# naver-ai/egtr

Measured on AMD Instinct MI355X. Metric: images/sec end-to-end SGG, 600x1000 input, N=200 queries, higher is better.
Workload: dtype f32; 1 GPU; VG inference: ResNet-50, N=200, 6 enc/6 dec, 150 classes, 50 predicates, 600x1000, bs=1/GPU fp32 (BASELINE configs[1]); hip_graph=True, gemm_tuning=True, miopen_find=True, parallelism=replicas x1 (independent images, no collective)

## Files before the change

### egtr_amd/csrc/conv3x3_x6.hip

```cpp
#include <hip/hip_runtime.h>
#include <stdint.h>

#include "common.h"
#include "x6_common.h"
#include "xs_format.h"

namespace {
using namespace x6;
typedef float f32x4v __attribute__((ext_vector_type(4)));

__device__ __forceinline__ f32x4v shift_relu(f32x4v v, f32x4v sh) {
  return f32x4v{egtr_relu(v.x + sh.x), egtr_relu(v.y + sh.y), egtr_relu(v.z + sh.z), egtr_relu(v.w + sh.w)};
}

struct ConvArgs {
  const float* x;
  const char* w;
  float* y;
  int B, H, W, N;
  int tiles_x, tiles_y;
  const float* in_shift;
};

#ifdef EGTR_CONV_TIMING
constexpr int kRecWg = 4096;
__device__ unsigned long long g_conv_rec[kRecWg][8];
#define CONV_T(v) const unsigned long long v = __builtin_amdgcn_s_memtime()
#else
#define CONV_T(v) do { } while (0)
#endif

template <int C, int TH, int WM, int NTW, int NWV = 4, bool SHIFT = false>
__global__ __launch_bounds__(64 * NWV) void conv3x3_x6_kernel(ConvArgs A) {
  constexpr int TW = 8;
  constexpr int HW_ = TW + 2, HH = TH + 2, HP = HH * HW_;
  constexpr int KC = C / 16;
  constexpr int KS = 9 * KC;
  constexpr int kPitch = C + 8;
  constexpr int MTW = (TH / 4) / WM;
  constexpr int WN = NWV / WM;
  constexpr int NT = 64 * NWV;
  constexpr int BN = 32 * NTW * WN;
#ifndef EGTR_CONV_PF
#define EGTR_CONV_PF 3
#endif
  constexpr int PF = EGTR_CONV_PF;
  constexpr int C4 = C / 4;
  static_assert(TH % (4 * WM) == 0 && NWV % WM == 0, "tile shape");
  extern __shared__ __attribute__((aligned(16))) char s_raw[];
  __bf16* const sA = reinterpret_cast<__bf16*>(s_raw);

  const int tid = threadIdx.x, lane = tid & 63, li = lane & 31, hf = lane >> 5;
  const int wave = __builtin_amdgcn_readfirstlane(tid >> 6);
  const int wm = wave / WN, wn = wave % WN;
#ifdef EGTR_CONV_TIMING
  const unsigned long long rt0 = __builtin_amdgcn_s_memrealtime();
#endif
  CONV_T(t0);
  const int nblocks = A.N / BN;
  int t = blockIdx.x;
  const int nb = t % nblocks;
  t /= nblocks;
  const int tx = t % A.tiles_x;
  t /= A.tiles_x;
  const int ty = t % A.tiles_y, b = t / A.tiles_y;
  const int y0 = ty * TH, x0 = tx * TW;
  const int nt0 = nb * (BN / 32) + wn * NTW;

  const char* const wlane = A.w + (size_t)nt0 * KS * (3 * xs::kFragBytes) + lane * 16;
  bf16x8 w[PF + 1][NTW][3];
  auto load_w = [&](int ks, bf16x8 (&dst)[NTW][3]) {
#pragma unroll
    for (int tt = 0; tt < NTW; ++tt)
#pragma unroll
      for (int p = 0; p < 3; ++p)
        dst[tt][p] = *reinterpret_cast<const bf16x8*>(wlane + ((size_t)(tt * KS + ks) * 3 + p) * xs::kFragBytes);
  };

  {
    constexpr float kPad = SHIFT ? -__builtin_inff() : 0.f;
    static_assert(!SHIFT || NT % C4 == 0, "one channel quad per thread");
    f32x4v sh = f32x4v{0.f, 0.f, 0.f, 0.f};
    if constexpr (SHIFT) sh = *reinterpret_cast<const f32x4v*>(A.in_shift + 4 * (tid % C4));
    constexpr int CHUNKS = HP * C4;
    constexpr int NQ = (CHUNKS + NT - 1) / NT;
    constexpr int CH = 6;
    const float* const xb = A.x + (size_t)b * A.H * A.W * C;
#pragma unroll
    for (int q0 = 0; q0 < NQ; q0 += CH) {
      f32x4v v[CH];
#pragma unroll
      for (int q = 0; q < CH; ++q) {
        const int idx = tid + NT * (q0 + q);
        const int hp = idx / C4, c4 = idx % C4;
        const int gy = y0 - 1 + hp / HW_, gx = x0 - 1 + hp % HW_;
        const bool in = (q0 + q < NQ) && idx < CHUNKS && gy >= 0 && gy < A.H && gx >= 0 && gx < A.W;
        v[q] = f32x4v{kPad, kPad, kPad, kPad};
        if (in) v[q] = *reinterpret_cast<const f32x4v*>(xb + ((size_t)gy * A.W + gx) * C + 4 * c4);
      }
      if (q0 == 0) {
        static_for<PF>([&](auto i_) {
          constexpr int i = decltype(i_)::value;
          load_w(i, w[i]);
        });
        __builtin_amdgcn_sched_barrier(0);
      }
#pragma unroll
      for (int q = 0; q < CH; ++q) {
        const int idx = tid + NT * (q0 + q);
        if (q0 + q < NQ && idx < CHUNKS) {
          const int hp = idx / C4, c4 = idx % C4;
          f32x4v u = v[q];
          if constexpr (SHIFT) u = shift_relu(u, sh);
          const xs::Split3 s0 = xs::split3_fast(u.x), s1 = xs::split3_fast(u.y), s2 = xs::split3_fast(u.z),
                           s3 = xs::split3_fast(u.w);
          __bf16* p = sA + hp * kPitch + 4 * c4;
          *reinterpret_cast<uint2*>(p) = make_uint2(xs::pack_hi16(s0.hi, s1.hi), xs::pack_hi16(s2.hi, s3.hi));
          *reinterpret_cast<uint2*>(p + HP * kPitch) = make_uint2(xs::pack_hi16(s0.mid, s1.mid), xs::pack_hi16(s2.mid, s3.mid));
          *reinterpret_cast<uint2*>(p + 2 * HP * kPitch) = make_uint2(xs::pack_hi16(s0.lo, s1.lo), xs::pack_hi16(s2.lo, s3.lo));
        }
      }
    }
  }
  CONV_T(t1);
  __syncthreads();
  CONV_T(t2);

  f32x16 acc[MTW][NTW];
#pragma unroll
  for (int m = 0; m < MTW; ++m)
#pragma unroll
    for (int tt = 0; tt < NTW; ++tt)
#pragma unroll
      for (int r = 0; r < 16; ++r) acc[m][tt][r] = 0.f;

  const __bf16* pa[MTW];
#pragma unroll
  for (int m = 0; m < MTW; ++m)
    pa[m] = sA + ((4 * (wm * MTW + m) + (li >> 3)) * HW_ + (li & 7)) * kPitch + 8 * hf;
  bf16x8 a[2][MTW][3];
  auto read_a = [&](auto ks_, bf16x8 (&dst)[MTW][3]) {
    constexpr int ks = decltype(ks_)::value;
    constexpr int tap = ks / KC, kc = ks % KC;
    constexpr int off = ((tap / 3) * HW_ + (tap % 3)) * kPitch + 16 * kc;
#pragma unroll
    for (int m = 0; m < MTW; ++m)
#pragma unroll
      for (int p = 0; p < 3; ++p) dst[m][p] = *reinterpret_cast<const bf16x8*>(pa[m] + p * HP * kPitch + off);
  };
  read_a(std::integral_constant<int, 0>{}, a[0]);
  static_for<KS>([&](auto ks_) {
    constexpr int ks = decltype(ks_)::value;
    if constexpr (ks + PF < KS) load_w(ks + PF, w[(ks + PF) % (PF + 1)]);
    if constexpr (ks + 1 < KS) read_a(std::integral_constant<int, ks + 1>{}, a[(ks + 1) & 1]);
    __builtin_amdgcn_sched_barrier(0);
#pragma unroll
    for (int m = 0; m < MTW; ++m)
#pragma unroll
      for (int tt = 0; tt < NTW; ++tt) acc[m][tt] = mfma6(a[ks & 1][m], w[ks % (PF + 1)][tt], acc[m][tt]);
    __builtin_amdgcn_sched_barrier(0);
  });

  CONV_T(t3);
  float* const yb = A.y + (size_t)b * A.H * A.W * A.N;
#pragma unroll
  for (int m = 0; m < MTW; ++m)
#pragma unroll
    for (int tt = 0; tt < NTW; ++tt) {
      const int col = (nt0 + tt) * 32 + li;
#pragma unroll
      for (int r = 0; r < 16; ++r) {
        const int p = (r & 3) + 8 * (r >> 2) + 4 * hf;
        const int gy = y0 + 4 * (wm * MTW + m) + (p >> 3), gx = x0 + (p & 7);
        if (gy < A.H && gx < A.W) yb[((size_t)gy * A.W + gx) * A.N + col] = acc[m][tt][r];
      }
    }
#ifdef EGTR_CONV_TIMING
  CONV_T(t4);
  asm volatile("s_waitcnt vmcnt(0)" ::: "memory");
  CONV_T(t5);
  if (tid == 0 && blockIdx.x < kRecWg) {
    unsigned long long* r = g_conv_rec[blockIdx.x];
    r[0] = rt0;
    r[1] = __builtin_amdgcn_s_memrealtime();
    r[2] = t1 - t0;
    r[3] = t2 - t1;
    r[4] = t3 - t2;
    r[5] = t4 - t3;
    r[6] = t5 - t4;
    r[7] = 1;
  }
#endif
}

template <int C, int CP, int STRIDE, int TAPS = 9, bool SHIFT = false>
__global__ __launch_bounds__(256) void conv3x3_x6_phased_kernel(ConvArgs A) {
  constexpr int TH = 4, TW = 8;
  static_assert(TAPS == 9 || TAPS == 1, "3x3 or 1x1");
  constexpr int HH = TAPS == 9 ? STRIDE * (TH - 1) + 3 : TH, HW_ = TAPS == 9 ? STRIDE * (TW - 1) + 3 : TW, HP = HH * HW_;
  constexpr int PH = C / CP;
  constexpr int KCP = CP / 16;
  constexpr int KSP = TAPS * KCP;
  constexpr int KS = PH * KSP;
  constexpr int kPitch = CP + 8;
  constexpr int PF = EGTR_CONV_PF;
  constexpr int C4 = CP / 4;
  static_assert(KSP % (PF + 1) == 0, "the fragment ring must line up at the phase boundary");
  static_assert(!SHIFT || (TAPS == 9 && 256 % C4 == 0), "one channel quad per thread");
  extern __shared__ __attribute__((aligned(16))) char s_raw[];
  __bf16* const sA = reinterpret_cast<__bf16*>(s_raw);

  const int tid = threadIdx.x, lane = tid & 63, li = lane & 31, hf = lane >> 5;
  const int wave = __builtin_amdgcn_readfirstlane(tid >> 6);
  const int nblocks = A.N / 128;
  int t = blockIdx.x;
  const int nb = t % nblocks;
  t /= nblocks;
  const int tx = t % A.tiles_x;
  t /= A.tiles_x;
  const int ty = t % A.tiles_y, b = t / A.tiles_y;
  const int y0 = ty * TH, x0 = tx * TW;
  const int iy0 = STRIDE * y0 - 1, ix0 = STRIDE * x0 - 1;
  const int nt = nb * 4 + wave;

  const char* const wlane = A.w + (size_t)nt * KS * (3 * xs::kFragBytes) + lane * 16;
  bf16x8 w[PF + 1][3];
  auto load_w = [&](int ks, bf16x8 (&dst)[3]) {
#pragma unroll
    for (int p = 0; p < 3; ++p) dst[p] = *reinterpret_cast<const bf16x8*>(wlane + ((size_t)ks * 3 + p) * xs::kFragBytes);
  };
  static_for<PF>([&](auto i_) {
    constexpr int i = decltype(i_)::value;
    load_w(i, w[i]);
  });
  __builtin_amdgcn_sched_barrier(0);

  f32x16 acc;
#pragma unroll
  for (int r = 0; r < 16; ++r) acc[r] = 0.f;
  const float* const xb = A.x + (size_t)b * A.H * A.W * C;
  constexpr int PS = TAPS == 9 ? STRIDE : 1;
  const __bf16* const pa = sA + (PS * (li >> 3) * HW_ + PS * (li & 7)) * kPitch + 8 * hf;

#pragma unroll 1
  for (int ph = 0; ph < PH; ++ph) {
    if (ph > 0) __syncthreads();
    {
      constexpr int CHUNKS = HP * C4;
      constexpr int NQ = (CHUNKS + 255) / 256;
      constexpr int CH = NQ < 8 ? NQ : 8;
      constexpr float kPad = SHIFT ? -__builtin_inff() : 0.f;
      f32x4v sh = f32x4v{0.f, 0.f, 0.f, 0.f};
      if constexpr (SHIFT) sh = *reinterpret_cast<const f32x4v*>(A.in_shift + ph * CP + 4 * (tid % C4));
#pragma unroll
      for (int q0 = 0; q0 < NQ; q0 += CH) {
        f32x4v v[CH];
#pragma unroll
        for (int q = 0; q < CH; ++q) {
          const int idx = tid + 256 * (q0 + q);
          const int hp = idx / C4, c4 = idx % C4;
          const int gy = TAPS == 9 ? iy0 + hp / HW_ : STRIDE * (y0 + hp / HW_), gx = TAPS == 9 ? ix0 + hp % HW_ : STRIDE * (x0 + hp % HW_);
          const bool in = (q0 + q < NQ) && idx < CHUNKS && gy >= 0 && gy < A.H && gx >= 0 && gx < A.W;
          v[q] = f32x4v{kPad, kPad, kPad, kPad};
          if (in) v[q] = *reinterpret_cast<const f32x4v*>(xb + ((size_t)gy * A.W + gx) * C + ph * CP + 4 * c4);
        }
#pragma unroll
        for (int q = 0; q < CH; ++q) {
          const int idx = tid + 256 * (q0 + q);
          if (q0 + q < NQ && idx < CHUNKS) {
            const int hp = idx / C4, c4 = idx % C4;
            f32x4v u = v[q];
            if constexpr (SHIFT) u = shift_relu(u, sh);
            const xs::Split3 s0 = xs::split3_fast(u.x), s1 = xs::split3_fast(u.y), s2 = xs::split3_fast(u.z),
                             s3 = xs::split3_fast(u.w);
            __bf16* p = sA + hp * kPitch + 4 * c4;
            *reinterpret_cast<uint2*>(p) = make_uint2(xs::pack_hi16(s0.hi, s1.hi), xs::pack_hi16(s2.hi, s3.hi));
            *reinterpret_cast<uint2*>(p + HP * kPitch) = make_uint2(xs::pack_hi16(s0.mid, s1.mid), xs::pack_hi16(s2.mid, s3.mid));
            *reinterpret_cast<uint2*>(p + 2 * HP * kPitch) = make_uint2(xs::pack_hi16(s0.lo, s1.lo), xs::pack_hi16(s2.lo, s3.lo));
          }
        }
      }
    }
    __syncthreads();

    const int ks0 = ph * KSP;
    bf16x8 a[2][3];
    auto read_a = [&](auto j_, bf16x8 (&dst)[3]) {
      constexpr int j = decltype(j_)::value;
      constexpr int tap = j / KCP, kc = j % KCP;
      constexpr int off = ((tap / 3) * HW_ + (tap % 3)) * kPitch + 16 * kc;
#pragma unroll
      for (int p = 0; p < 3; ++p) dst[p] = *reinterpret_cast<const bf16x8*>(pa + p * HP * kPitch + off);
    };
    read_a(std::integral_constant<int, 0>{}, a[0]);
    static_for<KSP>([&](auto j_) {
      constexpr int j = decltype(j_)::value;
      if (ks0 + j + PF < KS) load_w(ks0 + j + PF, w[(j + PF) % (PF + 1)]);
      if constexpr (j + 1 < KSP) read_a(std::integral_constant<int, j + 1>{}, a[(j + 1) & 1]);
      __builtin_amdgcn_sched_barrier(0);
      acc = mfma6(a[j & 1], w[j % (PF + 1)], acc);
      __builtin_amdgcn_sched_barrier(0);
    });
  }

  const int Ho = (A.H - 1) / STRIDE + 1, Wo = (A.W - 1) / STRIDE + 1;
  float* const yb = A.y + (size_t)b * Ho * Wo * A.N;
  const int col = nt * 32 + li;
#pragma unroll
  for (int r = 0; r < 16; ++r) {
    const int p = (r & 3) + 8 * (r >> 2) + 4 * hf;
    const int gy = y0 + (p >> 3), gx = x0 + (p & 7);
    if (gy < Ho && gx < Wo) yb[((size_t)gy * Wo + gx) * A.N + col] = acc[r];
  }
}

template <int C, int CP, int STRIDE, bool SHIFT = false>
__global__ __launch_bounds__(256) void conv3x3_x6_ksplit_kernel(ConvArgs A) {
  constexpr int TH = 4, TW = 8;
  constexpr int HH = STRIDE * (TH - 1) + 3, HW_ = STRIDE * (TW - 1) + 3, HP = HH * HW_;
  constexpr int PH = C / CP;
  constexpr int KCP = CP / 16;
  constexpr int KSP = 9 * KCP;
  constexpr int KCW = KCP / 4;
  constexpr int JS = 9 * KCW;
  constexpr int kPitch = CP + 8;
  constexpr int PF = (JS % 6 == 0) ? 5 : 2;
  constexpr int C4 = CP / 4;
  static_assert(KCP % 4 == 0 && JS % (PF + 1) == 0, "phase shape");
  static_assert(!SHIFT || 256 % C4 == 0, "one channel quad per thread");
  extern __shared__ __attribute__((aligned(16))) char s_raw[];
  __bf16* const sA = reinterpret_cast<__bf16*>(s_raw);

  const int tid = threadIdx.x, lane = tid & 63, li = lane & 31, hf = lane >> 5;
  const int wave = __builtin_amdgcn_readfirstlane(tid >> 6);
  const int ntiles = A.N / 32;
  int t = blockIdx.x;
  const int nt = t % ntiles;
  t /= ntiles;
  const int tx = t % A.tiles_x;
  t /= A.tiles_x;
  const int ty = t % A.tiles_y, b = t / A.tiles_y;
  const int y0 = ty * TH, x0 = tx * TW;
  const int iy0 = STRIDE * y0 - 1, ix0 = STRIDE * x0 - 1;

  const char* const wlane = A.w + (size_t)nt * (PH * KSP) * (3 * xs::kFragBytes) + lane * 16;
  auto wptr = [&](int ph, int j) {
    const int ks = ph * KSP + (j / KCW) * KCP + wave * KCW + (j % KCW);
    return wlane + (size_t)ks * 3 * xs::kFragBytes;
  };
  bf16x8 w[PF + 1][3];
  auto load_w = [&](int ph, int j, bf16x8 (&dst)[3]) {
    const char* p0 = wptr(ph, j);
#pragma unroll
    for (int p = 0; p < 3; ++p) dst[p] = *reinterpret_cast<const bf16x8*>(p0 + p * xs::kFragBytes);
  };
  static_for<PF>([&](auto i_) {
    constexpr int i = decltype(i_)::value;
    load_w(0, i, w[i]);
  });
  __builtin_amdgcn_sched_barrier(0);

  f32x16 acc;
#pragma unroll
  for (int r = 0; r < 16; ++r) acc[r] = 0.f;
  const float* const xb = A.x + (size_t)b * A.H * A.W * C;
  const __bf16* const pa = sA + (STRIDE * (li >> 3) * HW_ + STRIDE * (li & 7)) * kPitch + 8 * hf + 16 * KCW * wave;

#pragma unroll 1
  for (int ph = 0; ph < PH; ++ph) {
    if (ph > 0) __syncthreads();
    {
      constexpr int CHUNKS = HP * C4;
      constexpr int NQ = (CHUNKS + 255) / 256;
      constexpr int CH = NQ < 8 ? NQ : 8;
      constexpr float kPad = SHIFT ? -__builtin_inff() : 0.f;
      f32x4v sh = f32x4v{0.f, 0.f, 0.f, 0.f};
      if constexpr (SHIFT) sh = *reinterpret_cast<const f32x4v*>(A.in_shift + ph * CP + 4 * (tid % C4));
#pragma unroll
      for (int q0 = 0; q0 < NQ; q0 += CH) {
        f32x4v v[CH];
#pragma unroll
        for (int q = 0; q < CH; ++q) {
          const int idx = tid + 256 * (q0 + q);
          const int hp = idx / C4, c4 = idx % C4;
          const int gy = iy0 + hp / HW_, gx = ix0 + hp % HW_;
          const bool in = (q0 + q < NQ) && idx < CHUNKS && gy >= 0 && gy < A.H && gx >= 0 && gx < A.W;
          v[q] = f32x4v{kPad, kPad, kPad, kPad};
          if (in) v[q] = *reinterpret_cast<const f32x4v*>(xb + ((size_t)gy * A.W + gx) * C + ph * CP + 4 * c4);
        }
#pragma unroll
        for (int q = 0; q < CH; ++q) {
          const int idx = tid + 256 * (q0 + q);
          if (q0 + q < NQ && idx < CHUNKS) {
            const int hp = idx / C4, c4 = idx % C4;
            f32x4v u = v[q];
            if constexpr (SHIFT) u = shift_relu(u, sh);
            const xs::Split3 s0 = xs::split3_fast(u.x), s1 = xs::split3_fast(u.y), s2 = xs::split3_fast(u.z),
                             s3 = xs::split3_fast(u.w);
            __bf16* p = sA + hp * kPitch + 4 * c4;
            *reinterpret_cast<uint2*>(p) = make_uint2(xs::pack_hi16(s0.hi, s1.hi), xs::pack_hi16(s2.hi, s3.hi));
            *reinterpret_cast<uint2*>(p + HP * kPitch) = make_uint2(xs::pack_hi16(s0.mid, s1.mid), xs::pack_hi16(s2.mid, s3.mid));
            *reinterpret_cast<uint2*>(p + 2 * HP * kPitch) = make_uint2(xs::pack_hi16(s0.lo, s1.lo), xs::pack_hi16(s2.lo, s3.lo));
          }
        }
      }
    }
    __syncthreads();

    bf16x8 a[2][3];
    auto read_a = [&](auto j_, bf16x8 (&dst)[3]) {
      constexpr int j = decltype(j_)::value;
      constexpr int tap = j / KCW, kcl = j % KCW;
      constexpr int off = ((tap / 3) * HW_ + (tap % 3)) * kPitch + 16 * kcl;
#pragma unroll
      for (int p = 0; p < 3; ++p) dst[p] = *reinterpret_cast<const bf16x8*>(pa + p * HP * kPitch + off);
    };
    read_a(std::integral_constant<int, 0>{}, a[0]);
    static_for<JS>([&](auto j_) {
      constexpr int j = decltype(j_)::value;
      if constexpr (j + PF < JS) {
        load_w(ph, j + PF, w[(j + PF) % (PF + 1)]);
      } else {
        if (ph + 1 < PH) load_w(ph + 1, j + PF - JS, w[(j + PF) % (PF + 1)]);
      }
      if constexpr (j + 1 < JS) read_a(std::integral_constant<int, j + 1>{}, a[(j + 1) & 1]);
      __builtin_amdgcn_sched_barrier(0);
      acc = mfma6(a[j & 1], w[j % (PF + 1)], acc);
      __builtin_amdgcn_sched_barrier(0);
    });
  }

  __syncthreads();
  float* const part = reinterpret_cast<float*>(s_raw);
#pragma unroll
  for (int r = 0; r < 16; ++r) part[(wave * 16 + r) * 64 + lane] = acc[r];
  __syncthreads();
  const int Ho = (A.H - 1) / STRIDE + 1, Wo = (A.W - 1) / STRIDE + 1;
  float* const yb = A.y + (size_t)b * Ho * Wo * A.N;
  const int col = nt * 32 + li;
#pragma unroll
  for (int rr = 0; rr < 4; ++rr) {
    const int r = 4 * wave + rr;
    const float v = ((part[(0 * 16 + r) * 64 + lane] + part[(1 * 16 + r) * 64 + lane]) + part[(2 * 16 + r) * 64 + lane]) +
                    part[(3 * 16 + r) * 64 + lane];
    const int p = (r & 3) + 8 * (r >> 2) + 4 * hf;
    const int gy = y0 + (p >> 3), gx = x0 + (p & 7);
    if (gy < Ho && gx < Wo) yb[((size_t)gy * Wo + gx) * A.N + col] = v;
  }
}

template <int C, int CP, int STRIDE, bool SHIFT = false>
int launch_ksplit(hipStream_t st, ConvArgs A) {
  static unsigned long long raised = 0;
  constexpr int HP = (STRIDE * 3 + 3) * (STRIDE * 7 + 3);
  constexpr int lds = 3 * HP * (CP + 8) * 2;
  static_assert(lds >= 4 * 16 * 64 * 4, "the partial tiles reuse the halo tile's LDS");
  auto kern = conv3x3_x6_ksplit_kernel<C, CP, STRIDE, SHIFT>;
  if (lds > 64 * 1024) {
    const int rc = egtr_raise_dynamic_lds(reinterpret_cast<const void*>(kern), lds, &raised);
    if (rc != EGTR_OK) return rc;
  }
  const int Ho = (A.H - 1) / STRIDE + 1, Wo = (A.W - 1) / STRIDE + 1;
  A.tiles_x = (Wo + 7) / 8;
  A.tiles_y = (Ho + 3) / 4;
  const long long wgs = (long long)A.B * A.tiles_x * A.tiles_y * (A.N / 32);
  if (wgs >= (1ll << 31)) return EGTR_E_UNSUPPORTED;
  hipLaunchKernelGGL(kern, dim3((unsigned)wgs), dim3(256), lds, st, A);
  return egtr_check_launch();
}

template <int C, int CP, int STRIDE, int TAPS = 9, bool SHIFT = false>
int launch_phased(hipStream_t st, ConvArgs A) {
  static unsigned long long raised = 0;
  constexpr int HP = TAPS == 9 ? (STRIDE * 3 + 3) * (STRIDE * 7 + 3) : 32;
  constexpr int lds = 3 * HP * (CP + 8) * 2;
  auto kern = conv3x3_x6_phased_kernel<C, CP, STRIDE, TAPS, SHIFT>;
  if (lds > 64 * 1024) {
    const int rc = egtr_raise_dynamic_lds(reinterpret_cast<const void*>(kern), lds, &raised);
    if (rc != EGTR_OK) return rc;
  }
  const int Ho = (A.H - 1) / STRIDE + 1, Wo = (A.W - 1) / STRIDE + 1;
  A.tiles_x = (Wo + 7) / 8;
  A.tiles_y = (Ho + 3) / 4;
  const long long wgs = (long long)A.B * A.tiles_x * A.tiles_y * (A.N / 128);
  if (wgs >= (1ll << 31)) return EGTR_E_UNSUPPORTED;
  hipLaunchKernelGGL(kern, dim3((unsigned)wgs), dim3(256), lds, st, A);
  return egtr_check_launch();
}

template <int C, int TH, int WM, int NTW, int NWV = 4, bool SHIFT = false>
int launch(hipStream_t st, ConvArgs A) {
  static unsigned long long raised = 0;
  constexpr int lds = 3 * (TH + 2) * 10 * (C + 8) * 2;
  constexpr int BN = 32 * NTW * (NWV / WM);
  auto kern = conv3x3_x6_kernel<C, TH, WM, NTW, NWV, SHIFT>;
  if (lds > 64 * 1024) {
    const int rc = egtr_raise_dynamic_lds(reinterpret_cast<const void*>(kern), lds, &raised);
    if (rc != EGTR_OK) return rc;
  }
  A.tiles_x = (A.W + 7) / 8;
  A.tiles_y = (A.H + TH - 1) / TH;
  const long long wgs = (long long)A.B * A.tiles_x * A.tiles_y * (A.N / BN);
  if (wgs >= (1ll << 31)) return EGTR_E_UNSUPPORTED;
  hipLaunchKernelGGL(kern, dim3((unsigned)wgs), dim3(64 * NWV), lds, st, A);
  return egtr_check_launch();
}

}

#ifdef EGTR_CONV_TIMING
extern "C" int egtr_conv3x3_stamps(unsigned long long* host_out, int reset) {
  if (hipMemcpyFromSymbol(host_out, HIP_SYMBOL(g_conv_rec), sizeof(unsigned long long) * kRecWg * 8) != hipSuccess)
    return EGTR_E_LAUNCH;
  if (reset) {
    void* p = nullptr;
    if (hipGetSymbolAddress(&p, HIP_SYMBOL(g_conv_rec)) != hipSuccess ||
        hipMemset(p, 0, sizeof(unsigned long long) * kRecWg * 8) != hipSuccess)
      return EGTR_E_LAUNCH;
  }
  return EGTR_OK;
}
#endif

extern "C" int egtr_conv3x3_phase_channels(int C, int N, int stride, int variant) {
  if (C != N) return 0;
  if (stride == 1) {
    if (C == 64 || C == 128) return C;
    if (C == 256) return variant == 3 ? 256 : 128;
    if (C == 512) return 128;
    return 0;
  }
  if (stride == 2) return (C == 128 || C == 256 || C == 512) ? 64 : 0;
  return 0;
}

namespace {
template <bool SHIFT>
int conv3x3_dispatch(hipStream_t st, ConvArgs A, int C, int stride, int variant) {
  if (stride == 2) {
    if (C == 128) return variant == 1 ? launch_ksplit<128, 64, 2, SHIFT>(st, A) : launch_phased<128, 64, 2, 9, SHIFT>(st, A);
    if (C == 256) return variant == 1 ? launch_ksplit<256, 64, 2, SHIFT>(st, A) : launch_phased<256, 64, 2, 9, SHIFT>(st, A);
    if (variant == 1) return launch_phased<512, 64, 2, 9, SHIFT>(st, A);
    return launch_ksplit<512, 64, 2, SHIFT>(st, A);
  }
  if (C == 64) {
    if (variant == 1) return launch<64, 8, 2, 1, 4, SHIFT>(st, A);
    if (variant == 2) return launch<64, 16, 2, 1, 4, SHIFT>(st, A);
    if (variant == 3) return launch<64, 16, 4, 1, 4, SHIFT>(st, A);
    if (variant == 4) return launch_ksplit<64, 64, 1, SHIFT>(st, A);
    return launch<64, 4, 1, 1, 2, SHIFT>(st, A);
  }
  if (C == 128) {
    if (variant == 1) return launch<128, 8, 2, 1, 4, SHIFT>(st, A);
    if (variant == 3) return launch<128, 16, 4, 1, 4, SHIFT>(st, A);
    if (variant == 4) return launch<128, 4, 1, 1, 2, SHIFT>(st, A);
    if (variant == 2) return launch<128, 4, 1, 1, 4, SHIFT>(st, A);
    return launch_ksplit<128, 128, 1, SHIFT>(st, A);
  }
  if (C == 256) {
    if (variant == 1) return launch_phased<256, 128, 1, 9, SHIFT>(st, A);
    if (variant == 3) return launch<256, 4, 1, 1, 4, SHIFT>(st, A);
    return launch_ksplit<256, 128, 1, SHIFT>(st, A);
  }
  if (variant == 1) return launch_phased<512, 128, 1, 9, SHIFT>(st, A);
  return launch_ksplit<512, 128, 1, SHIFT>(st, A);
}

int conv3x3_check(const float* x, const void* w_xs, const float* y, int B, int H, int W, int C, int N, int stride, int variant) {
  if (!x || !w_xs || !y || B <= 0 || H <= 0 || W <= 0 || C <= 0 || N <= 0) return EGTR_E_ARG;
  if ((reinterpret_cast<uintptr_t>(x) & 15) || (reinterpret_cast<uintptr_t>(y) & 15) || (reinterpret_cast<uintptr_t>(w_xs) & 15))
    return EGTR_E_UNSUPPORTED;
  if (egtr_conv3x3_phase_channels(C, N, stride, variant) == 0) return EGTR_E_UNSUPPORTED;
  return EGTR_OK;
}
}

extern "C" int egtr_conv3x3_x6_f32(egtr_stream_t stream, const float* x, const void* w_xs, float* y, int B, int H, int W, int C,
                                   int N, int stride, int variant) {
  const int rc = conv3x3_check(x, w_xs, y, B, H, W, C, N, stride, variant);
  if (rc != EGTR_OK) return rc;
  ConvArgs A{x, static_cast<const char*>(w_xs), y, B, H, W, N, 0, 0, nullptr};
  return conv3x3_dispatch<false>(static_cast<hipStream_t>(stream), A, C, stride, variant);
}

extern "C" int egtr_conv3x3_x6_shift_f32(egtr_stream_t stream, const float* x, const float* in_shift, const void* w_xs, float* y,
                                         int B, int H, int W, int C, int N, int stride, int variant) {
  if (!in_shift) return EGTR_E_ARG;
  const int rc = conv3x3_check(x, w_xs, y, B, H, W, C, N, stride, variant);
  if (rc != EGTR_OK) return rc;
  if (reinterpret_cast<uintptr_t>(in_shift) & 15) return EGTR_E_UNSUPPORTED;
  ConvArgs A{x, static_cast<const char*>(w_xs), y, B, H, W, N, 0, 0, in_shift};
  return conv3x3_dispatch<true>(static_cast<hipStream_t>(stream), A, C, stride, variant);
}

extern "C" int egtr_conv1x1_strided_x6_f32(egtr_stream_t stream, const float* x, const void* w_xs, float* y, int B, int H, int W,
                                           int C, int N, int stride) {
  if (!x || !w_xs || !y || B <= 0 || H <= 0 || W <= 0 || C <= 0 || N <= 0) return EGTR_E_ARG;
  if ((reinterpret_cast<uintptr_t>(x) & 15) || (reinterpret_cast<uintptr_t>(y) & 15) || (reinterpret_cast<uintptr_t>(w_xs) & 15) ||
      N % 128 || (stride != 1 && stride != 2))
    return EGTR_E_UNSUPPORTED;
  ConvArgs A{x, static_cast<const char*>(w_xs), y, B, H, W, N, 0, 0, nullptr};
  hipStream_t st = static_cast<hipStream_t>(stream);
  if (stride == 2) {
    if (C == 256) return launch_phased<256, 256, 2, 1>(st, A);
    if (C == 512) return launch_phased<512, 256, 2, 1>(st, A);
    if (C == 1024) return launch_phased<1024, 256, 2, 1>(st, A);
    return EGTR_E_UNSUPPORTED;
  }
  if (C == 256) return launch_phased<256, 256, 1, 1>(st, A);
  if (C == 512) return launch_phased<512, 256, 1, 1>(st, A);
  if (C == 1024) return launch_phased<1024, 256, 1, 1>(st, A);
  return EGTR_E_UNSUPPORTED;
}
```

Measured before the change: 409.0 images/sec.

## Prefetch next channel phase's halo tile into registers during MFMA products

In the phased and k-split 3x3 conv kernels, when there are several channel phases, the global loads for the next phase's input halo are now issued in registers, spread across the MFMA steps of the current phase. They are parked into LDS (split to bf16x3) only after the products finish, which hides global-load latency behind the compute. Out-of-bounds loads are made branch-free by reading from a device pad constant. Launch bounds now request several workgroups per CU based on LDS size, and the k-split weight prefetch depth drops to 2 when there are multiple phases. The extra register-held tile raises register pressure, which may limit occupancy. Timing instrumentation is added under an ifdef.

```diff
diff --git a/egtr_amd/csrc/conv3x3_x6.hip b/egtr_amd/csrc/conv3x3_x6.hip
--- a/egtr_amd/csrc/conv3x3_x6.hip
+++ b/egtr_amd/csrc/conv3x3_x6.hip
@@ -26,6 +26,21 @@
 constexpr int kRecWg = 4096;
 __device__ unsigned long long g_conv_rec[kRecWg][8];
 #define CONV_T(v) const unsigned long long v = __builtin_amdgcn_s_memtime()
+__device__ __forceinline__ void conv_record_phased(unsigned long long rt0, unsigned long long tile0, unsigned long long park,
+                                                   unsigned long long prod, unsigned long long last, unsigned long long epi) {
+  asm volatile("s_waitcnt vmcnt(0)" ::: "memory");
+  if (threadIdx.x == 0 && blockIdx.x < kRecWg) {
+    unsigned long long* r = g_conv_rec[blockIdx.x];
+    r[0] = rt0;
+    r[1] = __builtin_amdgcn_s_memrealtime();
+    r[2] = tile0;
+    r[3] = park;
+    r[4] = prod;
+    r[5] = last;
+    r[6] = epi;
+    r[7] = 1;
+  }
+}
 #else
 #define CONV_T(v) do { } while (0)
 #endif
@@ -193,8 +208,66 @@
 #endif
 }
 
+__device__ const float g_conv_pad[8] = {0.f, 0.f, 0.f, 0.f, -__builtin_inff(), -__builtin_inff(), -__builtin_inff(), -__builtin_inff()};
+
+template <int C, int CP, int STRIDE, int TAPS, bool SHIFT>
+struct PhaseTile {
+  static constexpr int HH = TAPS == 9 ? STRIDE * 3 + 3 : 4, HW_ = TAPS == 9 ? STRIDE * 7 + 3 : 8, HP = HH * HW_;
+  static constexpr int C4 = CP / 4, kPitch = CP + 8;
+  static constexpr int CHUNKS = HP * C4;
+  static constexpr int NQ = (CHUNKS + 255) / 256;
+  f32x4v v[NQ];
+  f32x4v sh;
+
+  template <int q>
+  __device__ __forceinline__ void request(const ConvArgs& A, const float* xb, int y0, int x0, int tid, int ph) {
+    const int idx = tid + 256 * q;
+    const int hp = idx / C4, c4 = idx % C4;
+    const int gy = TAPS == 9 ? STRIDE * y0 - 1 + hp / HW_ : STRIDE * (y0 + hp / HW_);
+    const int gx = TAPS == 9 ? STRIDE * x0 - 1 + hp % HW_ : STRIDE * (x0 + hp % HW_);
+    const bool in = (idx < CHUNKS) & (gy >= 0) & (gy < A.H) & (gx >= 0) & (gx < A.W);
+    typedef const f32x4v __attribute__((address_space(1)))* gptr;
+    const gptr src = in ? (gptr)(xb + ((size_t)gy * A.W + gx) * C + ph * CP + 4 * c4) : (gptr)(g_conv_pad + (SHIFT ? 4 : 0));
+    v[q] = *src;
+  }
+  __device__ __forceinline__ void request_shift(const ConvArgs& A, int tid, int ph) {
+    if constexpr (SHIFT) sh = *reinterpret_cast<const f32x4v*>(A.in_shift + ph * CP + 4 * (tid % C4));
+  }
+  __device__ __forceinline__ void park(__bf16* sA, int tid) const {
+#pragma unroll
+    for (int q = 0; q < NQ; ++q) {
+      const int idx = tid + 256 * q;
+      if (idx < CHUNKS) {
+        const int hp = idx / C4, c4 = idx % C4;
+        f32x4v u = v[q];
+        if constexpr (SHIFT) u = shift_relu(u, sh);
+        const xs::Split3 s0 = xs::split3_fast(u.x), s1 = xs::split3_fast(u.y), s2 = xs::split3_fast(u.z),
+                         s3 = xs::split3_fast(u.w);
+        __bf16* p = sA + hp * kPitch + 4 * c4;
+        *reinterpret_cast<uint2*>(p) = make_uint2(xs::pack_hi16(s0.hi, s1.hi), xs::pack_hi16(s2.hi, s3.hi));
+        *reinterpret_cast<uint2*>(p + HP * kPitch) = make_uint2(xs::pack_hi16(s0.mid, s1.mid), xs::pack_hi16(s2.mid, s3.mid));
+        *reinterpret_cast<uint2*>(p + 2 * HP * kPitch) = make_uint2(xs::pack_hi16(s0.lo, s1.lo), xs::pack_hi16(s2.lo, s3.lo));
+      }
+    }
+  }
+  template <int STEPS>
+  static constexpr int per_step() { return (NQ + (STEPS + 1) / 2 - 1) / ((STEPS + 1) / 2); }
+};
+
+template <int C, int CP, int TAPS>
+constexpr bool phase_pipelined() {
+  return C / CP > 1 && !(TAPS == 9 && C == 128);
+}
+
+template <int C, int CP, int STRIDE, int TAPS, bool PIPE>
+constexpr int phase_wgs_per_cu() {
+  constexpr int lds = 3 * PhaseTile<C, CP, STRIDE, TAPS, false>::HP * (CP + 8) * 2;
+  return PIPE ? (160 * 1024) / lds : 1;
+}
+
 template <int C, int CP, int STRIDE, int TAPS = 9, bool SHIFT = false>
-__global__ __launch_bounds__(256) void conv3x3_x6_phased_kernel(ConvArgs A) {
+__global__ __launch_bounds__(256, (phase_wgs_per_cu<C, CP, STRIDE, TAPS, phase_pipelined<C, CP, TAPS>()>()))
+void conv3x3_x6_phased_kernel(ConvArgs A) {
   constexpr int TH = 4, TW = 8;
   static_assert(TAPS == 9 || TAPS == 1, "3x3 or 1x1");
   constexpr int HH = TAPS == 9 ? STRIDE * (TH - 1) + 3 : TH, HW_ = TAPS == 9 ? STRIDE * (TW - 1) + 3 : TW, HP = HH * HW_;
@@ -212,6 +285,10 @@
 
   const int tid = threadIdx.x, lane = tid & 63, li = lane & 31, hf = lane >> 5;
   const int wave = __builtin_amdgcn_readfirstlane(tid >> 6);
+#ifdef EGTR_CONV_TIMING
+  const unsigned long long rt0 = __builtin_amdgcn_s_memrealtime();
+#endif
+  CONV_T(t0);
   const int nblocks = A.N / 128;
   int t = blockIdx.x;
   const int nb = t % nblocks;
@@ -242,66 +319,131 @@
   constexpr int PS = TAPS == 9 ? STRIDE : 1;
   const __bf16* const pa = sA + (PS * (li >> 3) * HW_ + PS * (li & 7)) * kPitch + 8 * hf;
 
+#ifdef EGTR_CONV_TIMING
+  unsigned long long t_tile0 = 0, t_park = 0, t_prod = 0, t_last = 0;
+#endif
+  if constexpr (!phase_pipelined<C, CP, TAPS>()) {
 #pragma unroll 1
-  for (int ph = 0; ph < PH; ++ph) {
-    if (ph > 0) __syncthreads();
-    {
-      constexpr int CHUNKS = HP * C4;
-      constexpr int NQ = (CHUNKS + 255) / 256;
-      constexpr int CH = NQ < 8 ? NQ : 8;
-      constexpr float kPad = SHIFT ? -__builtin_inff() : 0.f;
-      f32x4v sh = f32x4v{0.f, 0.f, 0.f, 0.f};
-      if constexpr (SHIFT) sh = *reinterpret_cast<const f32x4v*>(A.in_shift + ph * CP + 4 * (tid % C4));
-#pragma unroll
-      for (int q0 = 0; q0 < NQ; q0 += CH) {
-        f32x4v v[CH];
-#pragma unroll
-        for (int q = 0; q < CH; ++q) {
-          const int idx = tid + 256 * (q0 + q);
-          const int hp = idx / C4, c4 = idx % C4;
-          const int gy = TAPS == 9 ? iy0 + hp / HW_ : STRIDE * (y0 + hp / HW_), gx = TAPS == 9 ? ix0 + hp % HW_ : STRIDE * (x0 + hp % HW_);
-          const bool in = (q0 + q < NQ) && idx < CHUNKS && gy >= 0 && gy < A.H && gx >= 0 && gx < A.W;
-          v[q] = f32x4v{kPad, kPad, kPad, kPad};
-          if (in) v[q] = *reinterpret_cast<const f32x4v*>(xb + ((size_t)gy * A.W + gx) * C + ph * CP + 4 * c4);
-        }
-#pragma unroll
-        for (int q = 0; q < CH; ++q) {
-          const int idx = tid + 256 * (q0 + q);
-          if (q0 + q < NQ && idx < CHUNKS) {
+    for (int ph = 0; ph < PH; ++ph) {
+      if (ph > 0) __syncthreads();
+      {
+        constexpr int CHUNKS = HP * C4;
+        constexpr int NQ = (CHUNKS + 255) / 256;
+        constexpr int CH = NQ < 8 ? NQ : 8;
+        constexpr float kPad = SHIFT ? -__builtin_inff() : 0.f;
+        f32x4v sh = f32x4v{0.f, 0.f, 0.f, 0.f};
+        if constexpr (SHIFT) sh = *reinterpret_cast<const f32x4v*>(A.in_shift + ph * CP + 4 * (tid % C4));
+#pragma unroll
+        for (int q0 = 0; q0 < NQ; q0 += CH) {
+          f32x4v v[CH];
+#pragma unroll
+          for (int q = 0; q < CH; ++q) {
+            const int idx = tid + 256 * (q0 + q);
             const int hp = idx / C4, c4 = idx % C4;
-            f32x4v u = v[q];
-            if constexpr (SHIFT) u = shift_relu(u, sh);
-            const xs::Split3 s0 = xs::split3_fast(u.x), s1 = xs::split3_fast(u.y), s2 = xs::split3_fast(u.z),
-                             s3 = xs::split3_fast(u.w);
-            __bf16* p = sA + hp * kPitch + 4 * c4;
-            *reinterpret_cast<uint2*>(p) = make_uint2(xs::pack_hi16(s0.hi, s1.hi), xs::pack_hi16(s2.hi, s3.hi));
-            *reinterpret_cast<uint2*>(p + HP * kPitch) = make_uint2(xs::pack_hi16(s0.mid, s1.mid), xs::pack_hi16(s2.mid, s3.mid));
-            *reinterpret_cast<uint2*>(p + 2 * HP * kPitch) = make_uint2(xs::pack_hi16(s0.lo, s1.lo), xs::pack_hi16(s2.lo, s3.lo));
+            const int gy = TAPS == 9 ? iy0 + hp / HW_ : STRIDE * (y0 + hp / HW_), gx = TAPS == 9 ? ix0 + hp % HW_ : STRIDE * (x0 + hp % HW_);
+            const bool in = (q0 + q < NQ) && idx < CHUNKS && gy >= 0 && gy < A.H && gx >= 0 && gx < A.W;
+            v[q] = f32x4v{kPad, kPad, kPad, kPad};
+            if (in) v[q] = *reinterpret_cast<const f32x4v*>(xb + ((size_t)gy * A.W + gx) * C + ph * CP + 4 * c4);
+          }
+#pragma unroll
+          for (int q = 0; q < CH; ++q) {
+            const int idx = tid + 256 * (q0 + q);
+            if (q0 + q < NQ && idx < CHUNKS) {
+              const int hp = idx / C4, c4 = idx % C4;
+              f32x4v u = v[q];
+              if constexpr (SHIFT) u = shift_relu(u, sh);
+              const xs::Split3 s0 = xs::split3_fast(u.x), s1 = xs::split3_fast(u.y), s2 = xs::split3_fast(u.z),
+                               s3 = xs::split3_fast(u.w);
+              __bf16* p = sA + hp * kPitch + 4 * c4;
+              *reinterpret_cast<uint2*>(p) = make_uint2(xs::pack_hi16(s0.hi, s1.hi), xs::pack_hi16(s2.hi, s3.hi));
+              *reinterpret_cast<uint2*>(p + HP * kPitch) = make_uint2(xs::pack_hi16(s0.mid, s1.mid), xs::pack_hi16(s2.mid, s3.mid));
+              *reinterpret_cast<uint2*>(p + 2 * HP * kPitch) = make_uint2(xs::pack_hi16(s0.lo, s1.lo), xs::pack_hi16(s2.lo, s3.lo));
+            }
           }
         }
       }
+      __syncthreads();
+
+      const int ks0 = ph * KSP;
+      bf16x8 a[2][3];
+      auto read_a = [&](auto j_, bf16x8 (&dst)[3]) {
+        constexpr int j = decltype(j_)::value;
+        constexpr int tap = j / KCP, kc = j % KCP;
+        constexpr int off = ((tap / 3) * HW_ + (tap % 3)) * kPitch + 16 * kc;
+#pragma unroll
+        for (int p = 0; p < 3; ++p) dst[p] = *reinterpret_cast<const bf16x8*>(pa + p * HP * kPitch + off);
+      };
+      read_a(std::integral_constant<int, 0>{}, a[0]);
+      static_for<KSP>([&](auto j_) {
+        constexpr int j = decltype(j_)::value;
+        if (ks0 + j + PF < KS) load_w(ks0 + j + PF, w[(j + PF) % (PF + 1)]);
+        if constexpr (j + 1 < KSP) read_a(std::integral_constant<int, j + 1>{}, a[(j + 1) & 1]);
+        __builtin_amdgcn_sched_barrier(0);
+        acc = mfma6(a[j & 1], w[j % (PF + 1)], acc);
+        __builtin_amdgcn_sched_barrier(0);
+      });
     }
+  } else {
+    using Tile = PhaseTile<C, CP, STRIDE, TAPS, SHIFT>;
+    auto products = [&](int ph, auto last_, auto& nx) {
+      constexpr bool LAST = decltype(last_)::value;
+      const int ks0 = ph * KSP;
+      bf16x8 a[2][3];
+      auto read_a = [&](auto j_, bf16x8 (&dst)[3]) {
+        constexpr int j = decltype(j_)::value;
+        constexpr int tap = j / KCP, kc = j % KCP;
+        constexpr int off = ((tap / 3) * HW_ + (tap % 3)) * kPitch + 16 * kc;
+#pragma unroll
+        for (int p = 0; p < 3; ++p) dst[p] = *reinterpret_cast<const bf16x8*>(pa + p * HP * kPitch + off);
+      };
+      read_a(std::integral_constant<int, 0>{}, a[0]);
+      static_for<KSP>([&](auto j_) {
+        constexpr int j = decltype(j_)::value;
+        if constexpr (!LAST || j + PF < KSP) load_w(ks0 + j + PF, w[(j + PF) % (PF + 1)]);
+        if constexpr (!LAST) {
+          constexpr int PER = Tile::template per_step<KSP>();
+          if constexpr (j == 0) nx.request_shift(A, tid, ph + 1);
+          static_for<PER>([&](auto i_) {
+            constexpr int q = j * PER + decltype(i_)::value;
+            if constexpr (q < Tile::NQ) nx.template request<q>(A, xb, y0, x0, tid, ph + 1);
+          });
+        }
+        if constexpr (j + 1 < KSP) read_a(std::integral_constant<int, j + 1>{}, a[(j + 1) & 1]);
+        __builtin_amdgcn_sched_barrier(0);
+        acc = mfma6(a[j & 1], w[j % (PF + 1)], acc);
+        __builtin_amdgcn_sched_barrier(0);
+      });
+    };
+    Tile nx;
+    nx.request_shift(A, tid, 0);
+    static_for<Tile::NQ>([&](auto q_) { nx.template request<decltype(q_)::value>(A, xb, y0, x0, tid, 0); });
+    nx.park(sA, tid);
     __syncthreads();
-
-    const int ks0 = ph * KSP;
-    bf16x8 a[2][3];
-    auto read_a = [&](auto j_, bf16x8 (&dst)[3]) {
-      constexpr int j = decltype(j_)::value;
-      constexpr int tap = j / KCP, kc = j % KCP;
-      constexpr int off = ((tap / 3) * HW_ + (tap % 3)) * kPitch + 16 * kc;
-#pragma unroll
-      for (int p = 0; p < 3; ++p) dst[p] = *reinterpret_cast<const bf16x8*>(pa + p * HP * kPitch + off);
-    };
-    read_a(std::integral_constant<int, 0>{}, a[0]);
-    static_for<KSP>([&](auto j_) {
-      constexpr int j = decltype(j_)::value;
-      if (ks0 + j + PF < KS) load_w(ks0 + j + PF, w[(j + PF) % (PF + 1)]);
-      if constexpr (j + 1 < KSP) read_a(std::integral_constant<int, j + 1>{}, a[(j + 1) & 1]);
-      __builtin_amdgcn_sched_barrier(0);
-      acc = mfma6(a[j & 1], w[j % (PF + 1)], acc);
-      __builtin_amdgcn_sched_barrier(0);
-    });
-  }
+    CONV_T(t1);
+#pragma unroll 1
+    for (int ph = 0; ph < PH - 1; ++ph) {
+      CONV_T(ta);
+      products(ph, std::false_type{}, nx);
+      CONV_T(tb);
+      __syncthreads();
+      nx.park(sA, tid);
+      __syncthreads();
+#ifdef EGTR_CONV_TIMING
+      t_prod += tb - ta;
+      t_park += __builtin_amdgcn_s_memtime() - tb;
+#endif
+    }
+    CONV_T(t2);
+    {
+      int none = 0;
+      products(PH - 1, std::true_type{}, none);
+    }
+    CONV_T(t3);
+#ifdef EGTR_CONV_TIMING
+    t_tile0 = t1 - t0, t_last = t3 - t2;
+#endif
+  }
+  CONV_T(te);
 
   const int Ho = (A.H - 1) / STRIDE + 1, Wo = (A.W - 1) / STRIDE + 1;
   float* const yb = A.y + (size_t)b * Ho * Wo * A.N;
@@ -312,10 +454,14 @@
     const int gy = y0 + (p >> 3), gx = x0 + (p & 7);
     if (gy < Ho && gx < Wo) yb[((size_t)gy * Wo + gx) * A.N + col] = acc[r];
   }
+#ifdef EGTR_CONV_TIMING
+  CONV_T(t4);
+  conv_record_phased(rt0, t_tile0, t_park, t_prod, t_last, t4 - te);
+#endif
 }
 
 template <int C, int CP, int STRIDE, bool SHIFT = false>
-__global__ __launch_bounds__(256) void conv3x3_x6_ksplit_kernel(ConvArgs A) {
+__global__ __launch_bounds__(256, (phase_wgs_per_cu<C, CP, STRIDE, 9, (C / CP > 1)>())) void conv3x3_x6_ksplit_kernel(ConvArgs A) {
   constexpr int TH = 4, TW = 8;
   constexpr int HH = STRIDE * (TH - 1) + 3, HW_ = STRIDE * (TW - 1) + 3, HP = HH * HW_;
   constexpr int PH = C / CP;
@@ -324,7 +470,7 @@
   constexpr int KCW = KCP / 4;
   constexpr int JS = 9 * KCW;
   constexpr int kPitch = CP + 8;
-  constexpr int PF = (JS % 6 == 0) ? 5 : 2;
+  constexpr int PF = (JS % 6 == 0 && PH == 1) ? 5 : 2;
   constexpr int C4 = CP / 4;
   static_assert(KCP % 4 == 0 && JS % (PF + 1) == 0, "phase shape");
   static_assert(!SHIFT || 256 % C4 == 0, "one channel quad per thread");
@@ -333,6 +479,10 @@
 
   const int tid = threadIdx.x, lane = tid & 63, li = lane & 31, hf = lane >> 5;
   const int wave = __builtin_amdgcn_readfirstlane(tid >> 6);
+#ifdef EGTR_CONV_TIMING
+  const unsigned long long rt0 = __builtin_amdgcn_s_memrealtime();
+#endif
+  CONV_T(t0);
   const int ntiles = A.N / 32;
   int t = blockIdx.x;
   const int nt = t % ntiles;
@@ -366,69 +516,137 @@
   const float* const xb = A.x + (size_t)b * A.H * A.W * C;
   const __bf16* const pa = sA + (STRIDE * (li >> 3) * HW_ + STRIDE * (li & 7)) * kPitch + 8 * hf + 16 * KCW * wave;
 
+#ifdef EGTR_CONV_TIMING
+  unsigned long long t_tile0 = 0, t_park = 0, t_prod = 0, t_last = 0;
+#endif
+  if constexpr (PH == 1) {
 #pragma unroll 1
-  for (int ph = 0; ph < PH; ++ph) {
-    if (ph > 0) __syncthreads();
-    {
-      constexpr int CHUNKS = HP * C4;
-      constexpr int NQ = (CHUNKS + 255) / 256;
-      constexpr int CH = NQ < 8 ? NQ : 8;
-      constexpr float kPad = SHIFT ? -__builtin_inff() : 0.f;
-      f32x4v sh = f32x4v{0.f, 0.f, 0.f, 0.f};
-      if constexpr (SHIFT) sh = *reinterpret_cast<const f32x4v*>(A.in_shift + ph * CP + 4 * (tid % C4));
-#pragma unroll
-      for (int q0 = 0; q0 < NQ; q0 += CH) {
-        f32x4v v[CH];
-#pragma unroll
-        for (int q = 0; q < CH; ++q) {
-          const int idx = tid + 256 * (q0 + q);
-          const int hp = idx / C4, c4 = idx % C4;
-          const int gy = iy0 + hp / HW_, gx = ix0 + hp % HW_;
-          const bool in = (q0 + q < NQ) && idx < CHUNKS && gy >= 0 && gy < A.H && gx >= 0 && gx < A.W;
-          v[q] = f32x4v{kPad, kPad, kPad, kPad};
-          if (in) v[q] = *reinterpret_cast<const f32x4v*>(xb + ((size_t)gy * A.W + gx) * C + ph * CP + 4 * c4);
-        }
-#pragma unroll
-        for (int q = 0; q < CH; ++q) {
-          const int idx = tid + 256 * (q0 + q);
-          if (q0 + q < NQ && idx < CHUNKS) {
+    for (int ph = 0; ph < PH; ++ph) {
+      if (ph > 0) __syncthreads();
+      {
+        constexpr int CHUNKS = HP * C4;
+        constexpr int NQ = (CHUNKS + 255) / 256;
+        constexpr int CH = NQ < 8 ? NQ : 8;
+        constexpr float kPad = SHIFT ? -__builtin_inff() : 0.f;
+        f32x4v sh = f32x4v{0.f, 0.f, 0.f, 0.f};
+        if constexpr (SHIFT) sh = *reinterpret_cast<const f32x4v*>(A.in_shift + ph * CP + 4 * (tid % C4));
+#pragma unroll
+        for (int q0 = 0; q0 < NQ; q0 += CH) {
+          f32x4v v[CH];
+#pragma unroll
+          for (int q = 0; q < CH; ++q) {
+            const int idx = tid + 256 * (q0 + q);
             const int hp = idx / C4, c4 = idx % C4;
-            f32x4v u = v[q];
-            if constexpr (SHIFT) u = shift_relu(u, sh);
-            const xs::Split3 s0 = xs::split3_fast(u.x), s1 = xs::split3_fast(u.y), s2 = xs::split3_fast(u.z),
-                             s3 = xs::split3_fast(u.w);
-            __bf16* p = sA + hp * kPitch + 4 * c4;
-            *reinterpret_cast<uint2*>(p) = make_uint2(xs::pack_hi16(s0.hi, s1.hi), xs::pack_hi16(s2.hi, s3.hi));
-            *reinterpret_cast<uint2*>(p + HP * kPitch) = make_uint2(xs::pack_hi16(s0.mid, s1.mid), xs::pack_hi16(s2.mid, s3.mid));
-            *reinterpret_cast<uint2*>(p + 2 * HP * kPitch) = make_uint2(xs::pack_hi16(s0.lo, s1.lo), xs::pack_hi16(s2.lo, s3.lo));
+            const int gy = iy0 + hp / HW_, gx = ix0 + hp % HW_;
+            const bool in = (q0 + q < NQ) && idx < CHUNKS && gy >= 0 && gy < A.H && gx >= 0 && gx < A.W;
+            v[q] = f32x4v{kPad, kPad, kPad, kPad};
+            if (in) v[q] = *reinterpret_cast<const f32x4v*>(xb + ((size_t)gy * A.W + gx) * C + ph * CP + 4 * c4);
+          }
+#pragma unroll
+          for (int q = 0; q < CH; ++q) {
+            const int idx = tid + 256 * (q0 + q);
+            if (q0 + q < NQ && idx < CHUNKS) {
+              const int hp = idx / C4, c4 = idx % C4;
+              f32x4v u = v[q];
+              if constexpr (SHIFT) u = shift_relu(u, sh);
+              const xs::Split3 s0 = xs::split3_fast(u.x), s1 = xs::split3_fast(u.y), s2 = xs::split3_fast(u.z),
+                               s3 = xs::split3_fast(u.w);
+              __bf16* p = sA + hp * kPitch + 4 * c4;
+              *reinterpret_cast<uint2*>(p) = make_uint2(xs::pack_hi16(s0.hi, s1.hi), xs::pack_hi16(s2.hi, s3.hi));
+              *reinterpret_cast<uint2*>(p + HP * kPitch) = make_uint2(xs::pack_hi16(s0.mid, s1.mid), xs::pack_hi16(s2.mid, s3.mid));
+              *reinterpret_cast<uint2*>(p + 2 * HP * kPitch) = make_uint2(xs::pack_hi16(s0.lo, s1.lo), xs::pack_hi16(s2.lo, s3.lo));
+            }
           }
         }
       }
+      __syncthreads();
+
+      bf16x8 a[2][3];
+      auto read_a = [&](auto j_, bf16x8 (&dst)[3]) {
+        constexpr int j = decltype(j_)::value;
+        constexpr int tap = j / KCW, kcl = j % KCW;
+        constexpr int off = ((tap / 3) * HW_ + (tap % 3)) * kPitch + 16 * kcl;
+#pragma unroll
+        for (int p = 0; p < 3; ++p) dst[p] = *reinterpret_cast<const bf16x8*>(pa + p * HP * kPitch + off);
+      };
+      read_a(std::integral_constant<int, 0>{}, a[0]);
+      static_for<JS>([&](auto j_) {
+        constexpr int j = decltype(j_)::value;
+        if constexpr (j + PF < JS) {
+          load_w(ph, j + PF, w[(j + PF) % (PF + 1)]);
+        } else {
+          if (ph + 1 < PH) load_w(ph + 1, j + PF - JS, w[(j + PF) % (PF + 1)]);
+        }
+        if constexpr (j + 1 < JS) read_a(std::integral_constant<int, j + 1>{}, a[(j + 1) & 1]);
+        __builtin_amdgcn_sched_barrier(0);
+        acc = mfma6(a[j & 1], w[j % (PF + 1)], acc);
+        __builtin_amdgcn_sched_barrier(0);
+      });
     }
+  } else {
+    using Tile = PhaseTile<C, CP, STRIDE, 9, SHIFT>;
+    auto products = [&](int ph, auto last_, auto& nx) {
+      constexpr bool LAST = decltype(last_)::value;
+      bf16x8 a[2][3];
+      auto read_a = [&](auto j_, bf16x8 (&dst)[3]) {
+        constexpr int j = decltype(j_)::value;
+        constexpr int tap = j / KCW, kcl = j % KCW;
+        constexpr int off = ((tap / 3) * HW_ + (tap % 3)) * kPitch + 16 * kcl;
+#pragma unroll
+        for (int p = 0; p < 3; ++p) dst[p] = *reinterpret_cast<const bf16x8*>(pa + p * HP * kPitch + off);
+      };
+      read_a(std::integral_constant<int, 0>{}, a[0]);
+      static_for<JS>([&](auto j_) {
+        constexpr int j = decltype(j_)::value;
+        if constexpr (j + PF < JS) {
+          load_w(ph, j + PF, w[(j + PF) % (PF + 1)]);
+        } else if constexpr (!LAST) {
+          load_w(ph + 1, j + PF - JS, w[(j + PF) % (PF + 1)]);
+        }
+        if constexpr (!LAST) {
+          constexpr int PER = Tile::template per_step<JS>();
+          if constexpr (j == 0) nx.request_shift(A, tid, ph + 1);
+          static_for<PER>([&](auto i_) {
+            constexpr int q = j * PER + decltype(i_)::value;
+            if constexpr (q < Tile::NQ) nx.template request<q>(A, xb, y0, x0, tid, ph + 1);
+          });
+        }
+        if constexpr (j + 1 < JS) read_a(std::integral_constant<int, j + 1>{}, a[(j + 1) & 1]);
+        __builtin_amdgcn_sched_barrier(0);
+        acc = mfma6(a[j & 1], w[j % (PF + 1)], acc);
+        __builtin_amdgcn_sched_barrier(0);
+      });
+    };
+    Tile nx;
+    nx.request_shift(A, tid, 0);
+    static_for<Tile::NQ>([&](auto q_) { nx.template request<decltype(q_)::value>(A, xb, y0, x0, tid, 0); });
+    nx.park(sA, tid);
     __syncthreads();
-
-    bf16x8 a[2][3];
-    auto read_a = [&](auto j_, bf16x8 (&dst)[3]) {
-      constexpr int j = decltype(j_)::value;
-      constexpr int tap = j / KCW, kcl = j % KCW;
-      constexpr int off = ((tap / 3) * HW_ + (tap % 3)) * kPitch + 16 * kcl;
-#pragma unroll
-      for (int p = 0; p < 3; ++p) dst[p] = *reinterpret_cast<const bf16x8*>(pa + p * HP * kPitch + off);
-    };
-    read_a(std::integral_constant<int, 0>{}, a[0]);
-    static_for<JS>([&](auto j_) {
-      constexpr int j = decltype(j_)::value;
-      if constexpr (j + PF < JS) {
-        load_w(ph, j + PF, w[(j + PF) % (PF + 1)]);
-      } else {
-        if (ph + 1 < PH) load_w(ph + 1, j + PF - JS, w[(j + PF) % (PF + 1)]);
-      }
-      if constexpr (j + 1 < JS) read_a(std::integral_constant<int, j + 1>{}, a[(j + 1) & 1]);
-      __builtin_amdgcn_sched_barrier(0);
-      acc = mfma6(a[j & 1], w[j % (PF + 1)], acc);
-      __builtin_amdgcn_sched_barrier(0);
-    });
-  }
+    CONV_T(t1);
+#pragma unroll 1
+    for (int ph = 0; ph < PH - 1; ++ph) {
+      CONV_T(ta);
+      products(ph, std::false_type{}, nx);
+      CONV_T(tb);
+      __syncthreads();
+      nx.park(sA, tid);
+      __syncthreads();
+#ifdef EGTR_CONV_TIMING
+      t_prod += tb - ta;
+      t_park += __builtin_amdgcn_s_memtime() - tb;
+#endif
+    }
+    CONV_T(t2);
+    {
+      int none = 0;
+      products(PH - 1, std::true_type{}, none);
+    }
+    CONV_T(t3);
+#ifdef EGTR_CONV_TIMING
+    t_tile0 = t1 - t0, t_last = t3 - t2;
+#endif
+  }
+  CONV_T(te);
 
   __syncthreads();
   float* const part = reinterpret_cast<float*>(s_raw);
@@ -447,6 +665,10 @@
     const int gy = y0 + (p >> 3), gx = x0 + (p & 7);
     if (gy < Ho && gx < Wo) yb[((size_t)gy * Wo + gx) * A.N + col] = v;
   }
+#ifdef EGTR_CONV_TIMING
+  CONV_T(t4);
+  conv_record_phased(rt0, t_tile0, t_park, t_prod, t_last, t4 - te);
+#endif
 }
 
 template <int C, int CP, int STRIDE, bool SHIFT = false>
```

Measured after the change: 410.3 images/sec, median of 6. No clear change (+0.3%).
